# RL4M/PCRLv2

Hardware: AMD Instinct MI355X
Metric: 3D crops/sec (64x64x32, b=32) pretrain step (higher is better)
Workload: dtype bf16; 1 GPU; C2: PCRLv23d pre-train step, 64x64x32 global views x2 + 6 local 16^3, b=32/GPU, fwd+bwd+SGD; global_batch=32, parallelism=dp1

## Files before the change

### include/pcrl_hip.h

```cpp
#ifndef PCRL_HIP_H
#define PCRL_HIP_H

#include <stddef.h>
#include <stdint.h>

#ifdef __cplusplus
extern "C" {
#endif

typedef void* pcrl_stream_t;

enum { PCRL_F32 = 0, PCRL_BF16 = 1 };
enum { PCRL_ACT_NONE = 0, PCRL_ACT_RELU = 1, PCRL_ACT_SIGMOID = 2, PCRL_ACT_SILU = 3 ,
       PCRL_ACT_ELU = 4  };
enum { PCRL_OK = 0, PCRL_EINVAL = -1, PCRL_ELAUNCH = -2, PCRL_EWORKSPACE = -3 };

#define PCRL_CONV_BM 128

const char* pcrl_version(void);
const char* pcrl_last_error(void);
int pcrl_zero(void* p, size_t bytes, pcrl_stream_t stream);

int pcrl_pack_conv3_weight(const float* w_ref, void* w_fwd, void* w_dgrad, int Co, int Ci, int dtype, pcrl_stream_t stream);
int pcrl_pack_convt_weight(const float* w_ref, void* w_fwd, void* w_dgrad, int Ci, int Co, int dtype, pcrl_stream_t stream);

int64_t pcrl_conv3d_k3_stats_rows(int N, int D, int H, int W, int Ci, int Co, int dtype);
int64_t pcrl_conv3d_k3_fwd_kernel(int N, int D, int H, int W, int Ci, int Co, int dtype);
int pcrl_conv3d_k3_fwd(const void* x, const void* wp, const float* bias, void* y, float* stats_partial,
                       int N, int D, int H, int W, int Ci, int Co, int dtype, pcrl_stream_t stream);
int64_t pcrl_conv3d_k3_fwd_ws_bytes(int N, int D, int H, int W, int Ci, int Co, int dtype);
int pcrl_conv3d_k3_fwd_ws(const void* x, const void* wp, const float* bias, void* y, float* stats_partial, void* ws, int64_t ws_bytes,
                          int N, int D, int H, int W, int Ci, int Co, int dtype, pcrl_stream_t stream);

int64_t pcrl_conv3d_k3_fwd_affine_fused(int N, int D, int H, int W, int Ci, int Co, int dtype);
int64_t pcrl_conv3d_k3_fwd_affine_ws_bytes(int N, int D, int H, int W, int Ci, int Co, int dtype);
int pcrl_conv3d_k3_fwd_affine(const void* x, const void* wp, const float* bias, const float* scale, const float* shift, void* a, void* ws,
                              int64_t ws_bytes, int N, int D, int H, int W, int Ci, int Co, int act, int dtype, pcrl_stream_t stream);

int64_t pcrl_conv3d_k3_dgrad_bnred_rows(int N, int D, int H, int W, int Ci, int Co, int act, int dtype);
int pcrl_conv3d_k3_dgrad_bnred(const void* dy, const void* wp_dgrad, void* dx, const void* bn_y, const float* scale, const float* shift,
                               const float* mean, const float* rstd, float* partial, int N, int D, int H, int W, int Ci, int Co, int act,
                               int dtype, pcrl_stream_t stream);

size_t pcrl_conv3d_k3_wgrad_ws_bytes(int N, int D, int H, int W, int Ci, int Co);
int pcrl_conv3d_k3_wgrad(const void* x, const void* dy, float* dw_ref, void* ws, size_t ws_bytes,
                         int N, int D, int H, int W, int Ci, int Co, int dtype, pcrl_stream_t stream);

int64_t pcrl_conv3d_k3_c1_stats_rows(int N, int D, int H, int W, int Co, int dtype);
int pcrl_conv3d_k3_c1_fwd(const float* x, const float* w_ref, const float* bias, void* y, float* stats_partial,
                          int N, int D, int H, int W, int Co, int dtype, pcrl_stream_t stream);
int pcrl_conv3d_k3_c1_fwd_affine(const float* x, const float* w_ref, const float* bias, const float* scale, const float* shift, void* a,
                                 int N, int D, int H, int W, int Co, int act, int dtype, pcrl_stream_t stream);
size_t pcrl_conv3d_k3_c1_wgrad_ws_bytes(int N, int D, int H, int W, int Co);
int pcrl_conv3d_k3_c1_wgrad(const float* x, const void* dy, float* dw_ref, void* ws, size_t ws_bytes,
                            int N, int D, int H, int W, int Co, int dtype, pcrl_stream_t stream);

int64_t pcrl_conv3d_to1_stats_rows(int N, int D, int H, int W, int C, int taps, int dtype);
size_t pcrl_conv3d_to1_fwd_ws_bytes(int N, int D, int H, int W, int C, int taps);
int pcrl_conv3d_to1_fwd(const void* x, const float* w_ref, const float* bias, float* y, float* stats_partial,
                        void* ws, size_t ws_bytes, int N, int D, int H, int W, int C, int taps, int dtype,
                        pcrl_stream_t stream);
int pcrl_conv3d_to1_dgrad(const float* dy, const float* w_ref, const void* add_src, void* dx,
                          int N, int D, int H, int W, int C, int taps, int dtype, pcrl_stream_t stream);
size_t pcrl_conv3d_to1_wgrad_ws_bytes(int N, int D, int H, int W, int C, int taps);
int pcrl_conv3d_to1_wgrad(const void* x, const float* dy, float* dw_ref, float* db, void* ws, size_t ws_bytes,
                          int N, int D, int H, int W, int C, int taps, int dtype, pcrl_stream_t stream);

int pcrl_convt3d_k2s2_fwd(const void* x, const void* wp_fwd, const float* bias, void* y,
                          int N, int D, int H, int W, int Ci, int Co, int dtype, pcrl_stream_t stream);
// ... 274 lines not shown
```

### pcrlv2_amd/config.py

```python
import os

import torch

_DTYPES = {"fp32": torch.float32, "float32": torch.float32, "f32": torch.float32,
           "bf16": torch.bfloat16, "bfloat16": torch.bfloat16}
_default = _DTYPES[os.environ.get("PCRL_DTYPE", "fp32").lower()]


def default_compute_dtype() -> torch.dtype:
    return _default


def set_default_compute_dtype(dt):
    global _default
    _default = _DTYPES[dt.lower()] if isinstance(dt, str) else dt
    if _default not in (torch.float32, torch.bfloat16):
        raise ValueError(f"compute dtype must be float32 or bfloat16, got {dt}")


DIRECT_PARAM_GRADS = os.environ.get("PCRL_AUTOGRAD_PARAM_GRADS", "0") != "1"

_ws = os.environ.get("PCRL_WGRAD_STREAM", "")
WGRAD_SIDE_STREAM_3D = _ws != "0"
WGRAD_SIDE_STREAM_2D = _ws != "0"

FWD_BRANCH_STREAM = os.environ.get("PCRL_BRANCH_STREAM", "1") != "0"

VIEW_STREAMS_2D = os.environ.get("PCRL_VIEW_STREAMS_2D", "1") != "0"

UPC_ZERO_SUM = True

EARLY_COMPOSED = True

MAX_STEPS_AHEAD = int(os.environ.get("PCRL_MAX_STEPS_AHEAD", "2"))

VIEW_STREAMS = os.environ.get("PCRL_VIEW_STREAMS", "1") != "0"

FOLD_GAP_GRAD = True

FOLD_POOL_GRAD = True

FUSE_APPLY_CONSUMERS = True
DGRAD_BNRED = os.environ.get("PCRL_DGRAD_BNRED", "1") != "0"

COMPOSE_UPCONV = os.environ.get("PCRL_COMPOSE_UPCONV", "1") != "0"

PROVISION_FACTOR = int(os.environ.get("PCRL_PROVISION_FACTOR", "2"))


VIEW_WGRAD_INLINE = True


PREPACK = True

FUSED_GRAD_SUM = True

# ... 4 lines not shown
```

### pcrlv2_amd/csrc/conv_wgrad.hip

```cpp
#include "internal.h"
#include <mutex>

namespace {

enum { WG_CONV3 = 0, WG_UP2 = 1, WG_PLAIN = 2, WG_CONV2D = 3, WG_UPC = 4 };

struct Wg2d {
  int Hs, Ws, KW, stride, pad, up, CiP, ntaps;
};

struct WgradParams {
  const void* u;
  const void* v;
  float* ws;
  Dims g;
  int64_t M;
  int Cu, Cv, taps;
  int64_t chunk;
  Wg2d q;
};

__device__ __forceinline__ int quad_sw(int row) { return ((row >> 1) & 1) | (((row >> 3) & 1) << 1); }

template <typename T> struct WTile;
// ... 328 lines not shown
    WG_STORE(cur ^ 1);
    __syncthreads();
  }
#undef WG_LOAD
#undef WG_LOAD2D
#undef WG_LOADUPC
#undef WG_LOAD3D
#undef WG_STORE

  float* __restrict__ out = p.ws + ((int64_t)blockIdx.z * p.taps + t) * (int64_t)p.Cu * p.Cv;
#pragma unroll
  for (int a = 0; a < 2; ++a)
#pragma unroll
    for (int b = 0; b < 2; ++b)
#pragma unroll
      for (int r = 0; r < 4; ++r) {
        const int i = i0 + wi * 32 + a * 16 + (lane >> 4) * 4 + r;
        const int j = j0 + wj * 32 + b * 16 + (lane & 15);
        if (i < p.Cu && j < p.Cv) out[(int64_t)i * p.Cv + j] = acc[a][b][r];
      }
}

constexpr int RED_IJ = 16;
__global__ void __launch_bounds__(256) wgrad_reduce_kernel(const float* __restrict__ ws, float* __restrict__ out,
                                                           int splits, int taps, int Cu, int Cv, int Cv_out, bool accumulate = false) {
  __shared__ float tile[RED_IJ * 64];
  __shared__ double part[256];
  const int64_t per = (int64_t)Cu * Cv;
  const int64_t n_out = (int64_t)Cu * Cv_out;
  const int64_t ij0 = (int64_t)blockIdx.x * RED_IJ;
  const int npairs = taps * RED_IJ;
  const int zg = npairs <= 128 ? 256 / npairs : 1;
  const int span = zg > 1 ? npairs * zg : npairs;
  for (int q0 = threadIdx.x; q0 < span; q0 += 256) {
    const int g = q0 / npairs, q = q0 - g * npairs;
    const int t = q / RED_IJ, l = q % RED_IJ;
    const int64_t ij = ij0 + l;
    double s = 0.0;
    if (ij < n_out) {
      const int i = (int)(ij / Cv_out), j = (int)(ij % Cv_out);
      const float* src = ws + (int64_t)t * per + (int64_t)i * Cv + j;
      const int64_t zs = (int64_t)taps * per;
      double a0 = 0.0, a1 = 0.0, a2 = 0.0, a3 = 0.0;
      int z = g;
      for (; z + 3 * zg < splits; z += 4 * zg) {
        a0 += (double)src[(int64_t)(z + 0 * zg) * zs];
        a1 += (double)src[(int64_t)(z + 1 * zg) * zs];
        a2 += (double)src[(int64_t)(z + 2 * zg) * zs];
        a3 += (double)src[(int64_t)(z + 3 * zg) * zs];
      }
      for (; z < splits; z += zg) a0 += (double)src[(int64_t)z * zs];
      s = (a0 + a1) + (a2 + a3);
    }
    if (zg > 1) part[q0] = s;
    else tile[l * taps + t] = (float)s;
  }
  if (zg > 1) {
    __syncthreads();
    if ((int)threadIdx.x < npairs) {
      double s = part[threadIdx.x];
      for (int k = 1; k < zg; ++k) s += part[k * npairs + threadIdx.x];
      tile[(threadIdx.x % RED_IJ) * taps + threadIdx.x / RED_IJ] = (float)s;
    }
  }
  __syncthreads();
  const int64_t base = ij0 * taps, lim = n_out * taps;
  for (int k = threadIdx.x; k < npairs; k += 256)
    if (base + k < lim) out[base + k] = accumulate ? out[base + k] + tile[k] : tile[k];
}

int launch_wgrad_reduce(const float* ws, float* out, int splits, int taps, int Cu, int Cv, int Cv_out, hipStream_t stream, bool accumulate = false) {
  if (taps < 1 || taps > 64) return pcrl_fail(PCRL_EINVAL, "wgrad_reduce: %d taps", taps);
  const int blocks = (int)(((int64_t)Cu * Cv_out + RED_IJ - 1) / RED_IJ);
  for (int rep = accumulate ? 1 : (int)g_hooks.reduce_repeat; rep > 0; --rep)
    hipLaunchKernelGGL(wgrad_reduce_kernel, dim3(blocks), dim3(256), 0, stream, ws, out, splits, taps, Cu, Cv, Cv_out, accumulate);
  return pcrl_check_launch("wgrad_reduce");
}

template <int ZG>
__global__ void __launch_bounds__(256) wgrad2d_reduce_kernel(const float* __restrict__ ws, float* __restrict__ out, int splits, int taps, int Cu,
                                                             int CiP, int Ci_out) {
  constexpr int NO = 256 / ZG;
  __shared__ double part[ZG][NO];
  const int64_t per = (int64_t)Cu * taps * CiP;
  const int64_t total = (int64_t)Cu * taps * Ci_out;
  const int o = threadIdx.x % NO, zg = threadIdx.x / NO;
  const int64_t idx = (int64_t)blockIdx.x * NO + o;
  double a = 0.0;
  int64_t dst = 0;
  if (idx < total) {
    const int ci = (int)(idx % Ci_out);
    const int64_t r = idx / Ci_out;
    const int t = (int)(r % taps), co = (int)(r / taps);
    const float* src = ws + ((int64_t)co * taps + t) * CiP + ci;
    dst = ((int64_t)co * Ci_out + ci) * taps + t;
    double a1 = 0.0, a2 = 0.0, a3 = 0.0;
    int z = zg;
    for (; z + 3 * ZG < splits; z += 4 * ZG) {
      const float v0 = src[(int64_t)z * per], v1 = src[(int64_t)(z + ZG) * per], v2 = src[(int64_t)(z + 2 * ZG) * per], v3 = src[(int64_t)(z + 3 * ZG) * per];
// ... 588 lines not shown
  splits = (steps + per - 1) / per;
  return SplitPlanUp2{(int)splits, per * 32};
}

struct SplitPlan {
  int splits;
  int64_t chunk;
};
SplitPlan plan_splits(int64_t M, int Cu, int Cv, int taps) {
  const int64_t tiles = (int64_t)((Cu + 63) / 64) * ((Cv + 63) / 64) * taps;
  const int64_t steps = (M + 31) / 32;
  int64_t splits = 2048 / tiles;
  if (splits < 1) splits = 1;
  const int64_t max_splits = (steps + 7) / 8;
  if (splits > max_splits) splits = max_splits;
  if (splits < 1) splits = 1;
  int64_t steps_per = (steps + splits - 1) / splits;
  splits = (steps + steps_per - 1) / steps_per;
  return SplitPlan{(int)splits, steps_per * 32};
}

template <int GEOM>
int run_wgrad(const void* u, const void* v, float* dw_ref, void* ws, size_t ws_bytes, Dims g, int Cu, int Cv, int taps,
              int dtype, hipStream_t stream, int Cv_out = -1, Wg2d q = Wg2d{0, 0, 1, 1, 0, 0, 1, 1}) {
  if (Cv_out < 0) Cv_out = Cv;
  const int64_t M = (int64_t)g.N * g.D * g.H * g.W;
  const SplitPlan sp = plan_splits(M, Cu, Cv, taps);
  const size_t need = (size_t)sp.splits * taps * Cu * Cv * sizeof(float);
  if (ws_bytes < need || !ws) return pcrl_fail(PCRL_EWORKSPACE, "wgrad: workspace %zu < %zu", ws_bytes, need);
  WgradParams p{u, v, (float*)ws, g, M, Cu, Cv, taps, sp.chunk, q};
  dim3 grid((unsigned)(((Cu + 63) / 64) * ((Cv + 63) / 64)), (unsigned)taps, (unsigned)sp.splits);
  if (dtype == PCRL_BF16) {
    if (g_hooks.wgrad_tr) hipLaunchKernelGGL((wgrad_kernel<bf16, GEOM, true>), grid, dim3(256), 4 * 32 * 128, stream, p);
    else hipLaunchKernelGGL((wgrad_kernel<bf16, GEOM, false>), grid, dim3(256), 4 * 32 * 128, stream, p);
  } else if (dtype == PCRL_F32) {
    hipLaunchKernelGGL((wgrad_kernel<float, GEOM, false>), grid, dim3(256), 4 * 32 * 256, stream, p);
  } else {
    return pcrl_fail(PCRL_EINVAL, "wgrad: bad dtype %d", dtype);
  }
  if (int e = pcrl_check_launch("wgrad")) return e;
  return launch_wgrad_reduce((const float*)ws, dw_ref, sp.splits, taps, Cu, Cv, Cv_out, stream);
}


bool scalar_brick_ok(int D, int H, int W, int C, int taps, int dtype) {
  return dtype == PCRL_BF16 && g_hooks.wgrad_tr && taps == 27 && D % 4 == 0 && H % 8 == 0 && W % 8 == 0 && C % 8 == 0;
}
int scalar_brick_blocks(int64_t nbricks, int C) {
  const int ytiles = (C + 63) / 64;
  int64_t nb = 512 / ytiles;
  if (nb > nbricks) nb = nbricks;
  if (nb < 1) nb = 1;
  return (int)nb;
}
size_t scalar_brick_ws_bytes(int N, int D, int H, int W, int C) {
  const int64_t nbricks = (int64_t)N * (D / 4) * (H / 8) * (W / 8);
  return 8192 + (size_t)scalar_brick_blocks(nbricks, C) * C * 32 * sizeof(float);
}
int scalar_brick_launch(const void* act, const float* sfield, float* dw_ref, char* ws, int N, int D, int H, int W, int C, int flip,
                        hipStream_t stream) {
  const int64_t nbricks = (int64_t)N * (D / 4) * (H / 8) * (W / 8);
  const int nb = scalar_brick_blocks(nbricks, C);
  const int per = (int)((nbricks + nb - 1) / nb);
  const int blocks = (int)((nbricks + per - 1) / per);
// ... 42 lines not shown
    else hipLaunchKernelGGL((wgrad_upc8_kernel<bf16, false>), grid, dim3(256), 2 * 9 * 32 * 128, stream, p);
  } else if (dtype == PCRL_F32) {
    hipLaunchKernelGGL((wgrad_upc8_kernel<float, false>), grid, dim3(256), 2 * 9 * 32 * 256, stream, p);
  } else {
    return pcrl_fail(PCRL_EINVAL, "upconv wgrad: bad dtype %d", dtype);
  }
  if (int e = pcrl_check_launch("upconv wgrad")) return e;
  return launch_wgrad_reduce((const float*)ws, dweff, sp.splits, 64, Co, Ci, Ci, stream, accumulate);
}

size_t pcrl_upc_wgrad3_ws_bytes(int N, int D, int H, int W, int Ci, int Co) {
  return (size_t)pcrl_wgrad_brick_upc_slabs(N, D, H, W, Ci, Co) * 27 * 8 * Co * Ci * sizeof(float);
}
static __global__ void __launch_bounds__(256) wgrad_reduce_upc_kernel(const float* __restrict__ ws, float* __restrict__ out, int splits, int Co, int Ci,
                                                               bool accumulate) {
  __shared__ float tile[64][9];
  const int i = blockIdx.y, p = i / Co, co = i - p * Co, j0 = blockIdx.x * 64;
  const int q = threadIdx.x >> 5, jl = threadIdx.x & 31;
  const int tap = (((p >> 2) & 1) + ((q >> 2) & 1)) * 9 + (((p >> 1) & 1) + ((q >> 1) & 1)) * 3 + ((p & 1) + (q & 1));
  const int64_t per = (int64_t)8 * Co * Ci, zs = 27 * per;
  const float* src = ws + (int64_t)tap * per + (int64_t)i * Ci + j0 + jl;
  double a0 = 0.0, a1 = 0.0;
  const bool ok0 = j0 + jl < Ci, ok1 = j0 + jl + 32 < Ci;
  for (int z = 0; z < splits; ++z) {
    if (ok0) a0 += (double)src[(int64_t)z * zs];
    if (ok1) a1 += (double)src[(int64_t)z * zs + 32];
  }
  tile[jl][q] = (float)a0;
  tile[jl + 32][q] = (float)a1;
  __syncthreads();
#pragma unroll
  for (int h = 0; h < 2; ++h) {
    const int j = h * 32 + (threadIdx.x >> 3), qq = threadIdx.x & 7;
    if (j0 + j < Ci) {
      float* dst = out + ((int64_t)co * Ci + j0 + j) * 64 + p * 8 + qq;
      *dst = accumulate ? *dst + tile[j][qq] : tile[j][qq];
    }
  }
}
int pcrl_upc_wgrad3_launch(const void* dy0, const void* x, float* dweff, void* ws, size_t ws_bytes, int N, int D, int H, int W, int Ci, int Co,
                           hipStream_t stream, bool accumulate) {
  const int splits = pcrl_wgrad_brick_upc_slabs(N, D, H, W, Ci, Co);
  const size_t need = (size_t)splits * 27 * 8 * Co * Ci * sizeof(float);
  if (!ws || ws_bytes < need) return pcrl_fail(PCRL_EWORKSPACE, "upconv wgrad (brick): workspace %zu < %zu", ws_bytes, need);
  if (int e = pcrl_wgrad_brick_upc_launch(x, dy0, (float*)ws, N, D, H, W, Ci, Co, stream)) return e;
  hipLaunchKernelGGL(wgrad_reduce_upc_kernel, dim3((unsigned)((Ci + 63) / 64), (unsigned)(8 * Co)), dim3(256), 0, stream, (const float*)ws, dweff, splits, Co,
                     Ci, accumulate);
  return pcrl_check_launch("upconv wgrad (brick, reduce)");
}

// ... 2 lines not shown
  return g_hooks.wgrad_impl == 0 && pcrl_wgrad_brick_eligible(N, D, H, W, Ci, Co, dtype) ? CONV3_WG_BRICK : CONV3_WG_GATHER;
}
enum ConvtWgradRoute { CONVT_WG_GATHER = 0, CONVT_WG_ALLTAPS };
static ConvtWgradRoute convt_wgrad_route(int Ci, int Co, int dtype) {
  return g_hooks.wgrad_impl == 0 && dtype == PCRL_BF16 && g_hooks.wgrad_tr && Ci % 64 == 0 && Co % 64 == 0 ? CONVT_WG_ALLTAPS : CONVT_WG_GATHER;
}
enum ScalarWgradRoute { SCALAR_WG_PLAIN = 0, SCALAR_WG_BRICK, SCALAR_WG_POINTWISE };
static ScalarWgradRoute scalar_wgrad_route(int D, int H, int W, int C, int taps, int dtype) {
  if (g_hooks.wgrad_impl != 0) return SCALAR_WG_PLAIN;
  if (scalar_brick_ok(D, H, W, C, taps, dtype)) return SCALAR_WG_BRICK;
  return taps == 1 && C % (dtype == PCRL_BF16 ? 8 : 4) == 0 && C <= 512 ? SCALAR_WG_POINTWISE : SCALAR_WG_PLAIN;
}

extern "C" size_t pcrl_conv3d_k3_wgrad_ws_bytes(int N, int D, int H, int W, int Ci, int Co) {
  const SplitPlan sp = plan_splits((int64_t)N * D * H * W, Co, Ci, 27);
  size_t a = (size_t)sp.splits * 27 * Co * Ci * sizeof(float);
  if (pcrl_wgrad_brick_eligible(N, D, H, W, Ci, Co, PCRL_BF16)) {
    const size_t b = (size_t)pcrl_wgrad_brick_splits(N, D, H, W, Ci, Co) * 27 * Co * Ci * sizeof(float);
    if (b > a) a = b;
  }
  return a;
}

extern "C" int pcrl_conv3d_k3_wgrad(const void* x, const void* dy, float* dw_ref, void* ws, size_t ws_bytes,
                                    int N, int D, int H, int W, int Ci, int Co, int dtype, pcrl_stream_t stream) {
  PCRL_REQUIRE(x && dy && dw_ref, "conv3d_k3_wgrad: null pointer");
  PCRL_REQUIRE(Ci > 0 && Co > 0 && Ci % 32 == 0 && Co % 32 == 0, "conv3d_k3_wgrad: channels must be multiples of 32 (Ci=%d Co=%d)", Ci, Co);
  if (conv3_wgrad_route(N, D, H, W, Ci, Co, dtype) == CONV3_WG_BRICK) {
    const int splits = pcrl_wgrad_brick_slabs(N, D, H, W, Ci, Co);
    const size_t need = (size_t)splits * 27 * Co * Ci * sizeof(float);
    if (!ws || ws_bytes < need) return pcrl_fail(PCRL_EWORKSPACE, "conv3d_k3_wgrad: workspace %zu < %zu", ws_bytes, need);
    if (int e = pcrl_wgrad_brick_launch(x, dy, (float*)ws, N, D, H, W, Ci, Co, as_stream(stream))) return e;
    return launch_wgrad_reduce((const float*)ws, dw_ref, splits, 27, Co, Ci, Ci, as_stream(stream));
  }
  return run_wgrad<WG_CONV3>(dy, x, dw_ref, ws, ws_bytes, Dims{N, D, H, W}, Co, Ci, 27, dtype, as_stream(stream));
}

extern "C" size_t pcrl_convt3d_k2s2_wgrad_ws_bytes(int N, int D, int H, int W, int Ci, int Co) {
  const int64_t M = (int64_t)N * D * H * W;
  const SplitPlan sp = plan_splits(M, Ci, Co, 8);
  size_t need = (size_t)sp.splits * 8 * Co * Ci * sizeof(float);
  if (Ci % 64 == 0 && Co % 64 == 0) {
    const size_t b = (size_t)plan_up2(M, Ci, Co).splits * 8 * Co * Ci * sizeof(float);
    if (b > need) need = b;
  }
  return need;
}

extern "C" int pcrl_convt3d_k2s2_wgrad(const void* x, const void* dy, float* dw_ref, void* ws, size_t ws_bytes,
                                       int N, int D, int H, int W, int Ci, int Co, int dtype, pcrl_stream_t stream) {
  PCRL_REQUIRE(x && dy && dw_ref, "convt3d_k2s2_wgrad: null pointer");
  PCRL_REQUIRE(Ci > 0 && Co > 0 && Ci % 32 == 0 && Co % 32 == 0, "convt3d_k2s2_wgrad: channels must be multiples of 32 (Ci=%d Co=%d)", Ci, Co);
  if (convt_wgrad_route(Ci, Co, dtype) == CONVT_WG_ALLTAPS) {
    const int64_t M = (int64_t)N * D * H * W;
    const SplitPlanUp2 sp = plan_up2(M, Ci, Co);
    const size_t need = (size_t)sp.splits * 8 * Co * Ci * sizeof(float);
    if (ws_bytes < need || !ws) return pcrl_fail(PCRL_EWORKSPACE, "convt3d_k2s2_wgrad: workspace %zu < %zu", ws_bytes, need);
    static std::once_flag attr_once;
// ... 205 lines not shown
```

### pcrlv2_amd/functions.py

```python
from __future__ import annotations

import weakref

import torch
from torch.autograd import Function

from . import config, ops
from ._lib import ACT_RELU, ACT_SIGMOID, ACT_SILU


def _act_grad(g, dtype):
    return ops.to_act(g, dtype)


_parked = {}
_parked_events = {}
_callback_queued = False
_final_callback = None
_finalize_hook = None


def set_ddp_callbacks(final_callback, finalize_hook):
    global _final_callback, _finalize_hook
    _final_callback, _finalize_hook = final_callback, finalize_hook
# ... 29 lines not shown
        torch.autograd.Variable._execution_engine.queue_callback(_end_of_backward)
        _callback_queued = True


def _park(p, g):
    global _callback_queued
    if g is None:
        return g
    if not config.DIRECT_PARAM_GRADS:
        ops.join_side_stream()
        return g
    if not p.requires_grad:
        return None
    _parked.setdefault(id(p), (p, []))[1].append(g)
    _queue_end_of_backward()
    return None


def reset_parked():
    global _callback_queued
    _parked.clear()
    _parked_events.clear()
    _callback_queued = False


def parked_params():
    return [p for p, _ in _parked.values()]


def take_parked(p):
    _parked_events.pop(id(p), None)
    return _parked.pop(id(p), (p, []))[1]


def _flush_fused(items):
    if not config.FUSED_GRAD_SUM:
        return False
    opt, idx = None, {}
    nsrc = 1
    for p, gs in items:
        slot = getattr(p, "_pcrl_gslot", None)
        if slot is None or p.grad is not None or (opt is not None and slot[0] is not opt) or len(gs) > 8:
            return False
        for g in gs:
            if not ops.is_shared_zero(g) and (g.dtype != torch.float32 or not g.is_contiguous() or g.numel() != p.numel() or g.data_ptr() % 4
                                              or g.device != p.device):
                return False
        opt = slot[0]
        idx[slot[1]] = (p, gs)
        nsrc = max(nsrc, len(gs))
    import ctypes
    t0, t1 = min(idx), max(idx) + 1
    srcs = (ctypes.c_void_p * ((t1 - t0) * nsrc))()
    for i, (p, gs) in idx.items():
        for k, g in enumerate(gs):
            if k == 0 or not ops.is_shared_zero(g):
                srcs[(i - t0) * nsrc + k] = g.data_ptr()
        p.grad = p._pcrl_gview
    ops.lib().call("pcrl_grad_sum", opt.flat_g, opt._offsets, opt._numels, ctypes.addressof(opt._offsets_c), ctypes.addressof(srcs), t0, t1 - t0, nsrc,
                   ops.stream_handle())
    return True


@torch.no_grad()
def flush_param_grads(params=None, on_stream=None):
    keys = list(_parked.keys()) if params is None else [id(p) for p in params if id(p) in _parked]
    items = [_parked.pop(k) for k in keys]
    if not items:
        return
    import contextlib
    ctx = contextlib.nullcontext()
    if on_stream is None:
        ops.join_side_stream()
    else:
        dev = items[0][0].device
        seen, missing = set(), False
        for k in keys:
            evs = _parked_events.pop(k, None)
            if evs is None:
                missing = True
                continue
            for ev in evs:
                if id(ev) not in seen:
                    seen.add(id(ev))
                    on_stream.wait_event(ev)
        side = ops.producer_streams(dev)[:1]
        if side and side[0].cuda_stream != on_stream.cuda_stream:
            on_stream.wait_stream(side[0])
# ... 16 lines not shown
                targets.append((p.grad, gs, 0))
                continue
            view = getattr(p, "_pcrl_gview", None)
            if view is not None:
                copy_dst.append(view)
                copy_src.append(gs[0])
                p.grad = view
            else:
                own = gs[0].is_contiguous() and gs[0].shape == p.shape and not ops.is_shared_zero(gs[0])
                p.grad = gs[0] if own else gs[0].reshape(p.shape).clone()
            targets.append((p.grad, gs, 1))
        if copy_dst:
            torch._foreach_copy_(copy_dst, copy_src)
        while True:
            pairs = [(t, gs[first + level]) for t, gs, first in targets if first + level < len(gs)]
            if not pairs:
                break
            pairs = [(t, g) for t, g in pairs if not ops.is_shared_zero(g)]
            if pairs:
                torch._foreach_add_([t for t, _ in pairs], [g for _, g in pairs])
            level += 1


def mark_final(ctx, params):
    if _final_callback is None:
        return
    ev = None
    for p in params:
        if id(p) in _parked and p.is_cuda:
            if ev is None:
                ev = torch.cuda.Event()
                ev.record()
            _parked_events.setdefault(id(p), []).append(ev)
    if getattr(ctx, "pass_idx", 1) == 0:
        for p in params:
            _final_callback(p)


def _slope(mod):
    return mod.activation.weight if getattr(mod, "_prelu", False) else None


def _park_slope(mod, sv):
    if sv.prelu is None or sv.dslope is None:
        return
    if not config.DIRECT_PARAM_GRADS:
        raise RuntimeError("act='prelu' needs config.DIRECT_PARAM_GRADS (the slope gradient is delivered by the engine, not by autograd)")
# ... 33 lines not shown
        ctx.below = _below_saved(mod, x)
        _remember_output(mod, sv, a)
        ctx.wref, ctx.gref = w_eff, gamma
        ctx.pass_idx = getattr(mod, "_pass_idx", 1)
        ctx.plist = (w, b, gamma, beta)
        ctx.set_materialize_grads(False)
        return a

    @staticmethod
    def backward(ctx, da):
        if da is None:
            return (None,) * 6
        sv = ctx.sv
        da = da.contiguous() if sv.kind == "to1" else _act_grad(da, ctx.dt)
        dx, dw, db, dg, dbeta = ops.luconv_backward(sv, da, ctx.wref, ctx.gref, ctx.mod._packed, ctx.dt,
                                                    need_dx=ctx.needs_input_grad[0] and sv.kind != "c1", bnred=ctx.below)
        if ctx.ci:
            ops.join_side_stream()
            dw = dw[:, :ctx.ci].contiguous()
            dx = None if dx is None else dx[:, :ctx.ci]
        _park_slope(ctx.mod, sv)
        w, b, gamma, beta = ctx.plist
        out = dx, _park(w, dw), _park(b, db), _park(gamma, dg), _park(beta, dbeta), None
        mark_final(ctx, ctx.plist)
        return out


class LUConvPoolFn(Function):

    @staticmethod
    def forward(ctx, x, w, b, gamma, beta, mod, pool_only=False):
        dt = mod.compute_dtype
        (a, p), sv = ops.luconv_forward(x, w, b, gamma, beta, mod.bn1.running_mean, mod.bn1.running_var, mod._packed, mod._act, dt, pooled=True,
                                        prelu=_slope(mod), pool_only=pool_only)
        mod._count_batch()
        ctx.sv, ctx.mod, ctx.dt = sv, mod, dt
        ctx.below = _below_saved(mod, x)
        ctx.wref, ctx.gref = w, gamma
        ctx.pass_idx = getattr(mod, "_pass_idx", 1)
        ctx.plist = (w, b, gamma, beta)
        ctx.set_materialize_grads(False)
        ctx.pool_only = a is None
        mod._last_saved = sv
        return p if a is None else (a, p)

    @staticmethod
    def backward(ctx, *grads):
        da, dp = (None, grads[0]) if ctx.pool_only else grads
        if da is None and dp is None:
            return (None,) * 7
        sv, dt = ctx.sv, ctx.dt
        N, D, H, W, _, Co = sv.geom
        pool_dp = None
        if dp is not None:
            dp = _act_grad(dp, dt)
            if da is None and sv.prelu is None and ops.bn_pool_ok(D, H, W, Co, dt):
                pool_dp = dp
            else:
                a = ops.prelu_forward(sv.z, sv.prelu, dt) if sv.prelu is not None else ops.bn_act_apply(sv.y, sv.scale, sv.shift, N * D * H * W, Co, sv.act, dt)
                dfull = ops.maxpool_backward(a, dp, dt)
                da = dfull if da is None else _act_grad(da, dt) + dfull
        elif da is not None:
            da = _act_grad(da, dt)
        dx, dw, db, dg, dbeta = ops.luconv_backward(sv, da, ctx.wref, ctx.gref, ctx.mod._packed, dt, need_dx=ctx.needs_input_grad[0],
                                                    pool_dp=pool_dp, bnred=ctx.below)
        _park_slope(ctx.mod, sv)
        w, b, gamma, beta = ctx.plist
        out = dx, _park(w, dw), _park(b, db), _park(gamma, dg), _park(beta, dbeta), None, None
        mark_final(ctx, ctx.plist)
        return out


class MaxPoolFn(Function):

    @staticmethod
    def forward(ctx, x, dt):
        ctx.x, ctx.dt = x, dt
        ctx.set_materialize_grads(False)
        return ops.maxpool_forward(x, dt)

    @staticmethod
    def backward(ctx, dy):
        if dy is None:
            return None, None
        return ops.maxpool_backward(ctx.x, _act_grad(dy, ctx.dt), ctx.dt), None


class UpStageFn(Function):

    @staticmethod
    def forward(ctx, x, up_w, up_b, w0, b0, g0, be0, w1, b1, g1, be1, bn_g, bn_b, p0_w, p0_b, p1_g, p1_b, p3_w, p3_b,
                dw_, db_, dg_, dbe_, mod):
# ... 408 lines not shown
```

### pcrlv2_amd/ops.py

```python
from __future__ import annotations

import collections
import os
import weakref

import torch

from . import config
from ._lib import ACT_NONE, ACT_RELU, ACT_SIGMOID, CONV_BM, PcrlError, dtype_code, lib, stream_handle

BN_EPS = 1e-5
BN_MOMENTUM = 0.1

_ws_cache: dict = {}


def workspace(nbytes: int, device, arena=None) -> torch.Tensor:
    if arena is None:
        arena = torch.cuda.current_stream(device).cuda_stream if device.type == "cuda" else 0
    key = (device.type, device.index, arena)
    t = _ws_cache.get(key)
    if t is None or t.numel() < nbytes:
        t = torch.empty(max(int(nbytes), 1 << 20), dtype=torch.uint8, device=device)
        _ws_cache[key] = t
    return t
# ... 59 lines not shown
        if side is None:
            side = _side_streams[key] = torch.cuda.Stream(device=self.device)
        side.wait_stream(torch.cuda.current_stream(self.device))
        for t in self.operands:
            t.record_stream(side)
        _side_pending[key] = True
        self._cm = torch.cuda.stream(side)
        self._cm.__enter__()
        return lambda nb: workspace(nb, self.device)

    def __exit__(self, *exc):
        if self.active:
            self._cm.__exit__(*exc)
        return False


class side_branch(side_wgrad):

    def __init__(self, device, *operands):
        self.device, self.operands = device, operands
        self.active = config.FWD_BRANCH_STREAM and device.type == "cuda"


_defer_join = 0


class deferred_join:

    def __enter__(self):
        global _defer_join
        _defer_join += 1

    def __exit__(self, *exc):
        global _defer_join
        _defer_join -= 1
        if _defer_join == 0:
            join_side_stream()
        return False


def end_of_forward_join():
    if _defer_join == 0:
        join_side_stream()


def join_side_stream(device=None):
    for key, pending in list(_side_pending.items()):
        if pending and (device is None or (device.type, device.index) == key):
            dev = torch.device(key[0], key[1])
            cur = torch.cuda.current_stream(dev)
            cur.wait_stream(_side_streams[key])
            if not any(cur.cuda_stream == vs.cuda_stream for vs in _view_streams.values()):
                _side_pending[key] = False
    if _views_active:
        for (dt_, di_, _name), vs in _view_streams.items():
            if device is None or (device.type, device.index) == (dt_, di_):
                cur = torch.cuda.current_stream(torch.device(dt_, di_))
                if cur.cuda_stream != vs.cuda_stream:
                    cur.wait_stream(vs)


def side_stream(device):
    key = (device.type, device.index)
    side = _side_streams.get(key)
    if side is None:
        side = _side_streams[key] = torch.cuda.Stream(device=device)
    return side


# ... 719 lines not shown
        dx = None
        if need_dx:
            dx = new_act(N, D, H, W, Ci, dtype, dev)
            L.call("pcrl_conv3d_to1_dgrad", dy, conv_w.detach(), dx_add, dx, N, D, H, W, Ci, 27, dtype_code(dtype), s)
        return dx, dw, db, dgamma, dbeta
    if da is not None:
        dims(da)
    if sv.gn is not None:
        dy, dgamma, dbeta = gn_act_backward(da, sv.gn[0], gamma.detach(), sv.gn[1], sv.act, dtype)
        db = _f32(Co, dev)
        nbc = L.call("pcrl_colsum_ws_bytes", M, Co)
        L.call("pcrl_colsum", dy, db, workspace(nbc, dev), nbc, M, Co, dtype_code(dtype), s)
    else:
        pre = take_pre_partial(sv, da) if (da_row_g is None and pool_dp is None) else None
        dy, dgamma, dbeta = bn_act_backward(da, sv.y, gamma.detach(), sv.mean, sv.rstd, sv.scale, sv.shift, M, Co, sv.act, dtype,
                                            row_g=da_row_g, pool_dp=pool_dp, pre_partial=pre)
    if sv.kind == "c1":
        nb = L.call("pcrl_conv3d_k3_c1_wgrad_ws_bytes", N, D, H, W, Co)
        L.call("pcrl_conv3d_k3_c1_wgrad", sv.x, dy, dw, workspace(nb, dev), nb, N, D, H, W, Co, dtype_code(dtype), s)
        return None, dw, db, dgamma, dbeta
    def weight_gradient():
        nbw = L.call("pcrl_conv3d_k3_wgrad_ws_bytes", N, D, H, W, Ci, Co)
        with side_wgrad(dev, sv.x, dy) as ws:
            L.call("pcrl_conv3d_k3_wgrad", sv.x, dy, dw, ws(nbw), nbw, N, D, H, W, Ci, Co, dtype_code(dtype), stream_handle())

    weight_gradient()
    dx = None
    if need_dx:
        _, wd = packed.get(conv_w, dtype)
        dx = new_act(N, D, H, W, Ci, dtype, dev)
        nb = L.call("pcrl_conv3d_k3_fwd_ws_bytes", N, D, H, W, Co, Ci, dtype_code(dtype))
        part = None
        if dx_colsum is not None:
            rows = L.call("pcrl_conv3d_k3_stats_rows", N, D, H, W, Co, Ci, dtype_code(dtype))
            part = _f32(rows * Ci * 2, dev)
        brows = 0
        if (bnred is not None and part is None and config.DGRAD_BNRED and bnred.gn is None and getattr(bnred, "prelu", None) is None and bnred.mean is not None
                and bnred.y.dtype == dtype and bnred.y.numel() == M * Ci):
            brows = L.call("pcrl_conv3d_k3_dgrad_bnred_rows", N, D, H, W, Co, Ci, bnred.act, dtype_code(dtype))
        if brows:
            bpart = _f32(brows * Ci * 2, dev)
            L.call("pcrl_conv3d_k3_dgrad_bnred", dy, wd, dx, bnred.y, bnred.scale, bnred.shift, bnred.mean, bnred.rstd, bpart,
                   N, D, H, W, Co, Ci, bnred.act, dtype_code(dtype), s)
            bnred.pre_partial = (bpart, brows, dx)
        else:
            L.call("pcrl_conv3d_k3_fwd_ws", dy, wd, None, dx, part, workspace(nb, dev) if nb else None, nb, N, D, H, W, Co, Ci, dtype_code(dtype), s)
        if part is not None:
# ... 613 lines not shown
```

Baseline: 1094 crops/s.

## Batch deferred conv3d weight-gradient split reductions into one multi-job kernel launch

The split-K weight-gradient reduction for each 3x3x3 conv is no longer launched right after its partial-sum kernel. A job record is stored through a thread-local defer hook, and the deferred reductions are flushed at stage ends, side-stream joins or grad flushes as a single batched kernel that maps blocks to jobs through a start table. Each deferred job gets its own slice of a per-stream arena so the partial buffers stay alive until the flush. The reduce loops are also unrolled (16-way and 8-way) to raise memory-level parallelism. The aim is fewer small kernel launches and better GPU fill, at the cost of extra workspace memory, more complex flush ordering, and a risk of stale or missing gradients if a flush point is missed.

```diff
diff --git a/include/pcrl_hip.h b/include/pcrl_hip.h
--- a/include/pcrl_hip.h
+++ b/include/pcrl_hip.h
@@ -45,6 +45,18 @@
 size_t pcrl_conv3d_k3_wgrad_ws_bytes(int N, int D, int H, int W, int Ci, int Co);
 int pcrl_conv3d_k3_wgrad(const void* x, const void* dy, float* dw_ref, void* ws, size_t ws_bytes,
                          int N, int D, int H, int W, int Ci, int Co, int dtype, pcrl_stream_t stream);
+
+typedef struct pcrl_wgrad_job {
+  const float* ws;
+  float* out;
+  int splits, taps, Cu, Cv, Cv_out, accumulate;
+} pcrl_wgrad_job;
+int pcrl_conv3d_k3_wgrad_pass1(const void* x, const void* dy, float* dw_ref, void* ws, size_t ws_bytes, pcrl_wgrad_job* job,
+                               int N, int D, int H, int W, int Ci, int Co, int dtype, pcrl_stream_t stream);
+int64_t pcrl_conv3d_k3_wgrad_splits(int N, int D, int H, int W, int Ci, int Co, int dtype);
+void pcrl_wgrad_defer(pcrl_wgrad_job* job);
+int pcrl_wgrad_reduce_batch(const pcrl_wgrad_job* jobs, int njobs, pcrl_stream_t stream);
+int pcrl_wgrad_reduce_one(const pcrl_wgrad_job* job, pcrl_stream_t stream);
 
 int64_t pcrl_conv3d_k3_c1_stats_rows(int N, int D, int H, int W, int Co, int dtype);
 int pcrl_conv3d_k3_c1_fwd(const float* x, const float* w_ref, const float* bias, void* y, float* stats_partial,
diff --git a/pcrlv2_amd/config.py b/pcrlv2_amd/config.py
--- a/pcrlv2_amd/config.py
+++ b/pcrlv2_amd/config.py
@@ -32,6 +32,8 @@
 
 EARLY_COMPOSED = True
 
+BATCHED_WGRAD_REDUCE = True
+
 MAX_STEPS_AHEAD = int(os.environ.get("PCRL_MAX_STEPS_AHEAD", "2"))
 
 VIEW_STREAMS = os.environ.get("PCRL_VIEW_STREAMS", "1") != "0"
diff --git a/pcrlv2_amd/csrc/conv_wgrad.hip b/pcrlv2_amd/csrc/conv_wgrad.hip
--- a/pcrlv2_amd/csrc/conv_wgrad.hip
+++ b/pcrlv2_amd/csrc/conv_wgrad.hip
@@ -374,13 +374,11 @@
 }
 
 constexpr int RED_IJ = 16;
-__global__ void __launch_bounds__(256) wgrad_reduce_kernel(const float* __restrict__ ws, float* __restrict__ out,
-                                                           int splits, int taps, int Cu, int Cv, int Cv_out, bool accumulate = false) {
-  __shared__ float tile[RED_IJ * 64];
-  __shared__ double part[256];
+__device__ __forceinline__ void wgrad_reduce_body(const float* __restrict__ ws, float* __restrict__ out, int splits, int taps, int Cu, int Cv, int Cv_out,
+                                                  bool accumulate, int64_t block, float* tile, double* part) {
   const int64_t per = (int64_t)Cu * Cv;
   const int64_t n_out = (int64_t)Cu * Cv_out;
-  const int64_t ij0 = (int64_t)blockIdx.x * RED_IJ;
+  const int64_t ij0 = block * RED_IJ;
   const int npairs = taps * RED_IJ;
   const int zg = npairs <= 128 ? 256 / npairs : 1;
   const int span = zg > 1 ? npairs * zg : npairs;
@@ -395,6 +393,18 @@
       const int64_t zs = (int64_t)taps * per;
       double a0 = 0.0, a1 = 0.0, a2 = 0.0, a3 = 0.0;
       int z = g;
+      for (; z + 15 * zg < splits; z += 16 * zg) {
+        float v[16];
+#pragma unroll
+        for (int u = 0; u < 16; ++u) v[u] = src[(int64_t)(z + u * zg) * zs];
+#pragma unroll
+        for (int u = 0; u < 16; u += 4) {
+          a0 += (double)v[u + 0];
+          a1 += (double)v[u + 1];
+          a2 += (double)v[u + 2];
+          a3 += (double)v[u + 3];
+        }
+      }
       for (; z + 3 * zg < splits; z += 4 * zg) {
         a0 += (double)src[(int64_t)(z + 0 * zg) * zs];
         a1 += (double)src[(int64_t)(z + 1 * zg) * zs];
@@ -420,6 +430,27 @@
   for (int k = threadIdx.x; k < npairs; k += 256)
     if (base + k < lim) out[base + k] = accumulate ? out[base + k] + tile[k] : tile[k];
 }
+__global__ void __launch_bounds__(256) wgrad_reduce_kernel(const float* __restrict__ ws, float* __restrict__ out,
+                                                           int splits, int taps, int Cu, int Cv, int Cv_out, bool accumulate = false) {
+  __shared__ float tile[RED_IJ * 64];
+  __shared__ double part[256];
+  wgrad_reduce_body(ws, out, splits, taps, Cu, Cv, Cv_out, accumulate, blockIdx.x, tile, part);
+}
+
+constexpr int RED_BATCH_MAX = 32;
+struct WgradReduceTable {
+  pcrl_wgrad_job job[RED_BATCH_MAX];
+  int start[RED_BATCH_MAX + 1];
+  int n;
+};
+__global__ void __launch_bounds__(256) wgrad_reduce_batch_kernel(const WgradReduceTable tb) {
+  __shared__ float tile[RED_IJ * 64];
+  __shared__ double part[256];
+  int k = 0;
+  while (k + 1 < tb.n && (int)blockIdx.x >= tb.start[k + 1]) ++k;
+  const pcrl_wgrad_job& jb = tb.job[k];
+  wgrad_reduce_body(jb.ws, jb.out, jb.splits, jb.taps, jb.Cu, jb.Cv, jb.Cv_out, jb.accumulate != 0, (int64_t)((int)blockIdx.x - tb.start[k]), tile, part);
+}
 
 int launch_wgrad_reduce(const float* ws, float* out, int splits, int taps, int Cu, int Cv, int Cv_out, hipStream_t stream, bool accumulate = false) {
   if (taps < 1 || taps > 64) return pcrl_fail(PCRL_EINVAL, "wgrad_reduce: %d taps", taps);
@@ -427,6 +458,11 @@
   for (int rep = accumulate ? 1 : (int)g_hooks.reduce_repeat; rep > 0; --rep)
     hipLaunchKernelGGL(wgrad_reduce_kernel, dim3(blocks), dim3(256), 0, stream, ws, out, splits, taps, Cu, Cv, Cv_out, accumulate);
   return pcrl_check_launch("wgrad_reduce");
+}
+int finish_or_defer(pcrl_wgrad_job* job, const float* ws, float* out, int splits, int taps, int Cu, int Cv, int Cv_out, hipStream_t stream) {
+  if (!job) return launch_wgrad_reduce(ws, out, splits, taps, Cu, Cv, Cv_out, stream);
+  *job = pcrl_wgrad_job{ws, out, splits, taps, Cu, Cv, Cv_out, 0};
+  return PCRL_OK;
 }
 
 template <int ZG>
@@ -1061,7 +1097,7 @@
 
 template <int GEOM>
 int run_wgrad(const void* u, const void* v, float* dw_ref, void* ws, size_t ws_bytes, Dims g, int Cu, int Cv, int taps,
-              int dtype, hipStream_t stream, int Cv_out = -1, Wg2d q = Wg2d{0, 0, 1, 1, 0, 0, 1, 1}) {
+              int dtype, hipStream_t stream, int Cv_out = -1, Wg2d q = Wg2d{0, 0, 1, 1, 0, 0, 1, 1}, pcrl_wgrad_job* job = nullptr) {
   if (Cv_out < 0) Cv_out = Cv;
   const int64_t M = (int64_t)g.N * g.D * g.H * g.W;
   const SplitPlan sp = plan_splits(M, Cu, Cv, taps);
@@ -1078,7 +1114,7 @@
     return pcrl_fail(PCRL_EINVAL, "wgrad: bad dtype %d", dtype);
   }
   if (int e = pcrl_check_launch("wgrad")) return e;
-  return launch_wgrad_reduce((const float*)ws, dw_ref, sp.splits, taps, Cu, Cv, Cv_out, stream);
+  return finish_or_defer(job, (const float*)ws, dw_ref, sp.splits, taps, Cu, Cv, Cv_out, stream);
 }
 
 
@@ -1167,10 +1203,27 @@
   const float* src = ws + (int64_t)tap * per + (int64_t)i * Ci + j0 + jl;
   double a0 = 0.0, a1 = 0.0;
   const bool ok0 = j0 + jl < Ci, ok1 = j0 + jl + 32 < Ci;
-  for (int z = 0; z < splits; ++z) {
-    if (ok0) a0 += (double)src[(int64_t)z * zs];
-    if (ok1) a1 += (double)src[(int64_t)z * zs + 32];
-  }
+  const int c0 = ok0 ? 0 : -(j0 + jl), c1 = ok1 ? 32 : c0;
+  int z = 0;
+  for (; z + 8 <= splits; z += 8) {
+    float v0[8], v1[8];
+#pragma unroll
+    for (int u = 0; u < 8; ++u) {
+      v0[u] = src[(int64_t)(z + u) * zs + c0];
+      v1[u] = src[(int64_t)(z + u) * zs + c1];
+    }
+#pragma unroll
+    for (int u = 0; u < 8; ++u) {
+      a0 += (double)v0[u];
+      a1 += (double)v1[u];
+    }
+  }
+  for (; z < splits; ++z) {
+    a0 += (double)src[(int64_t)z * zs + c0];
+    a1 += (double)src[(int64_t)z * zs + c1];
+  }
+  if (!ok0) a0 = 0.0;
+  if (!ok1) a1 = 0.0;
   tile[jl][q] = (float)a0;
   tile[jl + 32][q] = (float)a1;
   __syncthreads();
@@ -1219,18 +1272,65 @@
   return a;
 }
 
-extern "C" int pcrl_conv3d_k3_wgrad(const void* x, const void* dy, float* dw_ref, void* ws, size_t ws_bytes,
-                                    int N, int D, int H, int W, int Ci, int Co, int dtype, pcrl_stream_t stream) {
+static int conv3d_k3_wgrad_impl(const void* x, const void* dy, float* dw_ref, void* ws, size_t ws_bytes, int N, int D, int H, int W, int Ci, int Co, int dtype,
+                                hipStream_t stream, pcrl_wgrad_job* job) {
   PCRL_REQUIRE(x && dy && dw_ref, "conv3d_k3_wgrad: null pointer");
   PCRL_REQUIRE(Ci > 0 && Co > 0 && Ci % 32 == 0 && Co % 32 == 0, "conv3d_k3_wgrad: channels must be multiples of 32 (Ci=%d Co=%d)", Ci, Co);
   if (conv3_wgrad_route(N, D, H, W, Ci, Co, dtype) == CONV3_WG_BRICK) {
     const int splits = pcrl_wgrad_brick_slabs(N, D, H, W, Ci, Co);
     const size_t need = (size_t)splits * 27 * Co * Ci * sizeof(float);
     if (!ws || ws_bytes < need) return pcrl_fail(PCRL_EWORKSPACE, "conv3d_k3_wgrad: workspace %zu < %zu", ws_bytes, need);
-    if (int e = pcrl_wgrad_brick_launch(x, dy, (float*)ws, N, D, H, W, Ci, Co, as_stream(stream))) return e;
-    return launch_wgrad_reduce((const float*)ws, dw_ref, splits, 27, Co, Ci, Ci, as_stream(stream));
-  }
-  return run_wgrad<WG_CONV3>(dy, x, dw_ref, ws, ws_bytes, Dims{N, D, H, W}, Co, Ci, 27, dtype, as_stream(stream));
+    if (int e = pcrl_wgrad_brick_launch(x, dy, (float*)ws, N, D, H, W, Ci, Co, stream)) return e;
+    return finish_or_defer(job, (const float*)ws, dw_ref, splits, 27, Co, Ci, Ci, stream);
+  }
+  return run_wgrad<WG_CONV3>(dy, x, dw_ref, ws, ws_bytes, Dims{N, D, H, W}, Co, Ci, 27, dtype, stream, -1, Wg2d{0, 0, 1, 1, 0, 0, 1, 1}, job);
+}
+
+static thread_local pcrl_wgrad_job* t_defer_job = nullptr;
+extern "C" void pcrl_wgrad_defer(pcrl_wgrad_job* job) { t_defer_job = job; }
+
+extern "C" int pcrl_conv3d_k3_wgrad(const void* x, const void* dy, float* dw_ref, void* ws, size_t ws_bytes,
+                                    int N, int D, int H, int W, int Ci, int Co, int dtype, pcrl_stream_t stream) {
+  return conv3d_k3_wgrad_impl(x, dy, dw_ref, ws, ws_bytes, N, D, H, W, Ci, Co, dtype, as_stream(stream), t_defer_job);
+}
+extern "C" int pcrl_conv3d_k3_wgrad_pass1(const void* x, const void* dy, float* dw_ref, void* ws, size_t ws_bytes, pcrl_wgrad_job* job,
+                                          int N, int D, int H, int W, int Ci, int Co, int dtype, pcrl_stream_t stream) {
+  PCRL_REQUIRE(job, "conv3d_k3_wgrad_pass1: null job record");
+  return conv3d_k3_wgrad_impl(x, dy, dw_ref, ws, ws_bytes, N, D, H, W, Ci, Co, dtype, as_stream(stream), job);
+}
+extern "C" int64_t pcrl_conv3d_k3_wgrad_splits(int N, int D, int H, int W, int Ci, int Co, int dtype) {
+  if (conv3_wgrad_route(N, D, H, W, Ci, Co, dtype) == CONV3_WG_BRICK) return pcrl_wgrad_brick_slabs(N, D, H, W, Ci, Co);
+  return plan_splits((int64_t)N * D * H * W, Co, Ci, 27).splits;
+}
+
+extern "C" int pcrl_wgrad_reduce_one(const pcrl_wgrad_job* job, pcrl_stream_t stream) {
+  PCRL_REQUIRE(job && job->ws && job->out && job->splits >= 1 && job->Cu >= 1 && job->Cv >= 1 && job->Cv_out >= 1 && job->Cv_out <= job->Cv, "wgrad_reduce_one: bad job");
+  return launch_wgrad_reduce(job->ws, job->out, job->splits, job->taps, job->Cu, job->Cv, job->Cv_out, as_stream(stream), job->accumulate != 0);
+}
+
+extern "C" int pcrl_wgrad_reduce_batch(const pcrl_wgrad_job* jobs, int njobs, pcrl_stream_t stream) {
+  PCRL_REQUIRE(njobs >= 0 && (jobs || njobs == 0), "wgrad_reduce_batch: bad arguments");
+  for (int j0 = 0; j0 < njobs; j0 += RED_BATCH_MAX) {
+    WgradReduceTable tb;
+    tb.n = njobs - j0 < RED_BATCH_MAX ? njobs - j0 : RED_BATCH_MAX;
+    int64_t total = 0;
+    bool acc = false;
+    for (int k = 0; k < tb.n; ++k) {
+      const pcrl_wgrad_job& jb = jobs[j0 + k];
+      PCRL_REQUIRE(jb.ws && jb.out && jb.splits >= 1 && jb.Cu >= 1 && jb.Cv >= 1 && jb.Cv_out >= 1 && jb.Cv_out <= jb.Cv, "wgrad_reduce_batch: bad job %d", j0 + k);
+      if (jb.taps < 1 || jb.taps > 64) return pcrl_fail(PCRL_EINVAL, "wgrad_reduce_batch: job %d has %d taps", j0 + k, jb.taps);
+      tb.job[k] = jb;
+      tb.start[k] = (int)total;
+      total += ((int64_t)jb.Cu * jb.Cv_out + RED_IJ - 1) / RED_IJ;
+      acc = acc || jb.accumulate != 0;
+    }
+    PCRL_REQUIRE(total < ((int64_t)1 << 31), "wgrad_reduce_batch: %lld blocks", (long long)total);
+    for (int k = tb.n; k <= RED_BATCH_MAX; ++k) tb.start[k] = (int)total;
+    for (int rep = acc ? 1 : (int)g_hooks.reduce_repeat; rep > 0; --rep)
+      hipLaunchKernelGGL(wgrad_reduce_batch_kernel, dim3((unsigned)total), dim3(256), 0, as_stream(stream), tb);
+    if (int e = pcrl_check_launch("wgrad_reduce_batch")) return e;
+  }
+  return PCRL_OK;
 }
 
 extern "C" size_t pcrl_convt3d_k2s2_wgrad_ws_bytes(int N, int D, int H, int W, int Ci, int Co) {
diff --git a/pcrlv2_amd/functions.py b/pcrlv2_amd/functions.py
--- a/pcrlv2_amd/functions.py
+++ b/pcrlv2_amd/functions.py
@@ -75,6 +75,7 @@
     _parked.clear()
     _parked_events.clear()
     _callback_queued = False
+    ops.drop_wgrad_batch()
 
 
 def parked_params():
@@ -117,6 +118,7 @@
 
 @torch.no_grad()
 def flush_param_grads(params=None, on_stream=None):
+    ops.flush_wgrad_batch()
     keys = list(_parked.keys()) if params is None else [id(p) for p in params if id(p) in _parked]
     items = [_parked.pop(k) for k in keys]
     if not items:
@@ -179,7 +181,9 @@
             level += 1
 
 
-def mark_final(ctx, params):
+def mark_final(ctx, params, stage_end=True):
+    if stage_end:
+        ops.flush_wgrad_batch()
     if _final_callback is None:
         return
     ev = None
@@ -259,7 +263,7 @@
         _park_slope(ctx.mod, sv)
         w, b, gamma, beta = ctx.plist
         out = dx, _park(w, dw), _park(b, db), _park(gamma, dg), _park(beta, dbeta), None
-        mark_final(ctx, ctx.plist)
+        mark_final(ctx, ctx.plist, stage_end=ctx.below is None)
         return out
 
 
@@ -304,7 +308,7 @@
         _park_slope(ctx.mod, sv)
         w, b, gamma, beta = ctx.plist
         out = dx, _park(w, dw), _park(b, db), _park(gamma, dg), _park(beta, dbeta), None, None
-        mark_final(ctx, ctx.plist)
+        mark_final(ctx, ctx.plist, stage_end=ctx.below is None)
         return out
 
 
diff --git a/pcrlv2_amd/ops.py b/pcrlv2_amd/ops.py
--- a/pcrlv2_amd/ops.py
+++ b/pcrlv2_amd/ops.py
@@ -1,6 +1,7 @@
 from __future__ import annotations
 
 import collections
+import ctypes
 import os
 import weakref
 
@@ -106,6 +107,92 @@
         self.active = config.FWD_BRANCH_STREAM and device.type == "cuda"
 
 
+class WgradJob(ctypes.Structure):
+    _fields_ = [("ws", ctypes.c_void_p), ("out", ctypes.c_void_p), ("splits", ctypes.c_int), ("taps", ctypes.c_int), ("Cu", ctypes.c_int),
+                ("Cv", ctypes.c_int), ("Cv_out", ctypes.c_int), ("accumulate", ctypes.c_int)]
+
+
+class SlabArena:
+    ALIGN = 256
+
+    def __init__(self, alloc):
+        self.alloc, self.buf, self.off, self.extra, self.high = alloc, None, 0, [], 0
+
+    def take(self, nbytes: int):
+        n = (max(int(nbytes), 1) + self.ALIGN - 1) // self.ALIGN * self.ALIGN
+        if self.buf is None and not self.extra:
+            self.buf = self.alloc(max(n, self.high))
+        start = self.off
+        self.off += n
+        self.high = max(self.high, self.off)
+        if self.buf is not None and start + n <= self.buf.numel():
+            return self.buf.data_ptr() + start, start
+        self.extra.append(self.alloc(n))
+        return self.extra[-1].data_ptr(), None
+
+    def reset(self):
+        if self.extra or (self.buf is not None and self.buf.numel() < self.high):
+            self.buf = None
+        self.extra, self.off = [], 0
+
+
+class WgradBatch:
+    CAP = 64
+
+    def __init__(self, device, stream):
+        self.device, self.stream = device, stream
+        self.jobs, self.n, self.outs = (WgradJob * self.CAP)(), 0, []
+        self.arena = SlabArena(lambda nb: torch.empty(nb, dtype=torch.uint8, device=device))
+
+    def first_pass(self, name, out, nbytes, args_before, args_after):
+        if self.n == self.CAP:
+            self.flush()
+        L = lib()
+        ws, _ = self.arena.take(nbytes)
+        defer = L.fn["pcrl_wgrad_defer"][0]
+        defer(ctypes.addressof(self.jobs[self.n]))
+        try:
+            L.call(name, *args_before, out, ws, nbytes, *args_after)
+        finally:
+            defer(None)
+        self.n += 1
+        self.outs.append(out)
+
+    def flush(self):
+        if self.n:
+            n, self.n = self.n, 0
+            self.outs = []
+            lib().call("pcrl_wgrad_reduce_batch", ctypes.addressof(self.jobs), n, self.stream)
+        self.arena.reset()
+
+    def drop(self):
+        self.n, self.outs = 0, []
+        self.arena.reset()
+
+
+_wgrad_batches: dict = {}
+
+
+def wgrad_batch(device) -> WgradBatch:
+    h = stream_handle()
+    key = (device.type, device.index, h)
+    b = _wgrad_batches.get(key)
+    if b is None:
+        b = _wgrad_batches[key] = WgradBatch(device, h)
+    return b
+
+
+def flush_wgrad_batch():
+    for b in _wgrad_batches.values():
+        if b.n:
+            b.flush()
+
+
+def drop_wgrad_batch():
+    for b in _wgrad_batches.values():
+        b.drop()
+
+
 _defer_join = 0
 
 
@@ -129,6 +216,7 @@
 
 
 def join_side_stream(device=None):
+    flush_wgrad_batch()
     for key, pending in list(_side_pending.items()):
         if pending and (device is None or (device.type, device.index) == key):
             dev = torch.device(key[0], key[1])
@@ -894,7 +982,10 @@
     def weight_gradient():
         nbw = L.call("pcrl_conv3d_k3_wgrad_ws_bytes", N, D, H, W, Ci, Co)
         with side_wgrad(dev, sv.x, dy) as ws:
-            L.call("pcrl_conv3d_k3_wgrad", sv.x, dy, dw, ws(nbw), nbw, N, D, H, W, Ci, Co, dtype_code(dtype), stream_handle())
+            if config.BATCHED_WGRAD_REDUCE and dev.type == "cuda":
+                wgrad_batch(dev).first_pass("pcrl_conv3d_k3_wgrad", dw, nbw, (sv.x, dy), (N, D, H, W, Ci, Co, dtype_code(dtype), stream_handle()))
+            else:
+                L.call("pcrl_conv3d_k3_wgrad", sv.x, dy, dw, ws(nbw), nbw, N, D, H, W, Ci, Co, dtype_code(dtype), stream_handle())
 
     weight_gradient()
     dx = None
```

Measured after the change: 1101 crops/s (median of 6 runs). About the same (+0.6%).
